# ShinobuAmasaki/forgex

Measured on NVIDIA B200. Metric: input_GBps, higher is better.
Workload: dtype u8

## Files before the change

forgex_b200/csrc/fx_cabi.cu:

```cuda
#include <cuda_runtime.h>

#include <algorithm>
#include <atomic>
#include <cstdio>
#include <cstdlib>
#include <cstring>
#include <mutex>
#include <new>
#include <string>
#include <vector>

#include "../../include/forgex_b200.h"
#include "fx_internal.hpp"
#include "fx_kernels.cuh"

using namespace fxk;

namespace {

std::atomic<long long> g_launches{0};

constexpr int STATE_CAP = 16383;
constexpr int SPARSE_STATE_CAP = 2048;
constexpr int DIRECT_LIMIT_BYTES = 40 * 1024;
// ... 470 lines not shown
        if (spt < 32) spt = 32;
        if (spt > 2048) spt = 2048;
    }
    t.spt = (int)spt;
    t.cap = (int)cap;
    t.ntiles = (n + spt - 1) / spt;
    t.smem = (size_t)tile_offset(t.table_smem, t.spt) + (size_t)extra + (size_t)t.cap + 64;
    return t;
}

template <int OP, int KIND>
int launch_ragged_t(fx_pattern* p, const Plan& pl, const uint8_t* buf, const int64_t* off, int64_t n, int64_t total,
                    uint8_t* out, cudaStream_t s, int generic) {
    auto kern = k_bool_ragged<OP, KIND>;
    Tiling t = make_tiling(pl, n, total);
    int bps = 0;
    int rc = occupancy_grid(kern, 256, t.smem, p->dev.sm_count, bps);
    if (rc) return rc;
    long long cap = (long long)p->dev.sm_count * bps;
    int grid = (int)(t.ntiles < cap ? t.ntiles : cap);
    if (grid < 1) grid = 1;
    kern<<<grid, 256, t.smem, s>>>(pl.kp, buf, off, n, total, out, t.spt, t.cap, t.ntiles, t.table_smem, generic);
    g_launches++;
    return cuda_status(cudaGetLastError());
}

template <int KIND, int NR, bool HIGH, bool TWO>
int launch_sparse_t(fx_pattern* p, const Plan& pl, const SparseParams& sp, int table_bytes, const uint8_t* buf,
                    const int64_t* off, int64_t n, int64_t total, uint8_t* out, cudaStream_t s, int64_t stride) {
    auto kern = k_in_sparse<KIND, NR, HIGH, TWO>;
    int64_t avg = n > 0 ? (total + n - 1) / n : 1;
    if (avg < 1) avg = 1;
    int64_t want = (24 * 1024) / avg;
    const int spt = (int)(want < 32 ? 32 : want > 4096 ? 4096 : want);
    const int64_t ntiles = (n + spt - 1) / spt;
    const int table_smem = KIND == 3 ? 0 : (table_bytes + 15) & ~15;
    const size_t smem = (size_t)sparse_shared_head(table_smem) + 8 * (size_t)SPARSE_WARP_BYTES;
    int bps = 0;
    int rc = occupancy_grid(kern, 256, smem, p->dev.sm_count, bps);
    if (rc) return rc;
    long long cap = (long long)p->dev.sm_count * bps;
    long long wantg = (ntiles + 7) / 8;
    int grid = (int)(wantg < cap ? wantg : cap);
    if (grid < 1) grid = 1;
    const int prezeroed = sp.start_nul == 0 && pl.kp.q0_accepting == 0;
    if (prezeroed) CUDA_TRY(cudaMemsetAsync(out, 0, (size_t)n, s));
    kern<<<grid, 256, smem, s>>>(pl.kp, sp, buf, off, n, total, out, spt, ntiles, table_smem, prezeroed, stride);
    g_launches++;
    return cuda_status(cudaGetLastError());
}

template <int KIND, bool HIGH>
int launch_sparse_k(fx_pattern* p, const Plan& pl, const SparseParams& sp, int tb, const uint8_t* buf, const int64_t* off,
                    int64_t n, int64_t total, uint8_t* out, cudaStream_t s, int64_t stride) {
    if (p->first.sweep_nr == 1 && p->first.sweep_lo[0] == p->first.sweep_hi[0]) {
        const SparseParams& one = sp;
        if (p->first.two) return launch_sparse_t<KIND, -1, HIGH, true>(p, pl, one, tb, buf, off, n, total, out, s, stride);
        return launch_sparse_t<KIND, -1, HIGH, false>(p, pl, one, tb, buf, off, n, total, out, s, stride);
    }
    switch (p->first.sweep_nr) {
        case 0: return launch_sparse_t<KIND, 0, true, false>(p, pl, sp, tb, buf, off, n, total, out, s, stride);
        case 1: return launch_sparse_t<KIND, 1, HIGH, false>(p, pl, sp, tb, buf, off, n, total, out, s, stride);
        case 2: return launch_sparse_t<KIND, 2, HIGH, false>(p, pl, sp, tb, buf, off, n, total, out, s, stride);
        case 3: return launch_sparse_t<KIND, 3, HIGH, false>(p, pl, sp, tb, buf, off, n, total, out, s, stride);
        default: return launch_sparse_t<KIND, 4, HIGH, false>(p, pl, sp, tb, buf, off, n, total, out, s, stride);
    }
}

void fill_sweep(const FirstSet& f, SparseParams& sp) {
    for (int r = 0; r < 4; r++) {
        const int k = r < f.sweep_nr ? r : 0;
        sp.add_lo[r] = (0x80u - f.sweep_lo[k]) * 0x01010101u;
        sp.add_hi[r] = (0x7Fu - f.sweep_hi[k]) * 0x01010101u;
    }
    if (f.sweep_nr == 1 && f.sweep_lo[0] == f.sweep_hi[0]) sp.add_lo[0] = f.sweep_lo[0] * 0x01010101u;
    sp.second = f.second * 0x01010101u;
    sp.second_high = f.second_high ? 0xFFFFFFFFu : 0u;
}

int launch_sparse(fx_pattern* p, const Plan& pl, const uint8_t* buf, const int64_t* off, int64_t n, int64_t total,
// ... 1107 lines not shown
```

forgex_b200/csrc/fx_kernels.cuh:

```cuda
#pragma once
#include <cuda_runtime.h>
#include <stdint.h>

namespace fxk {

static constexpr uint32_t W_ACC = 0x8000u, W_INTER = 0x4000u, W_STATE = 0x3FFFu;
static constexpr uint32_t SF_ACC = 1, SF_END = 2, SF_INTER = 4, SF_MATCHED = 8, SF_FAILACC1 = 16;

struct KParams {
    const uint16_t* table;
    const uint8_t* classmap;
    const uint8_t* flags;
    const uint8_t* lits;
    int table_words;
    int nstates;
    int row_shift;
    int start, start_nul, q0, q0_accepting;
    int all_len, pre_len, suf_len;
    int all_active;
    int pre_active, suf_active;
    const uint16_t* a_table;
    const uint8_t* a_classmap;
    const uint8_t* a_flags;
    int a_row_shift, a_start_nul, a_q0;
// ... 756 lines not shown
            if (generic || r1 == OFF_BEYOND) {
                const int64_t o0 = __ldg(offsets + c.first + i), o1 = __ldg(offsets + c.first + i + 1);
                r = eval_bool_slow<OP>(p, buf + o0, o1 - o0);
            } else {
                const int len = r1 - r0;
                const uint32_t a = tile_addr + (uint32_t)r0;
                if (degenerate_text<OP>(len, len ? lds_u8(a) : 0)) r = p.q0_accepting != 0;
                else {
                    uint32_t high = 0;
                    r = result_flag(p, walk_smem(T, (uint32_t)p.start, a, len, high));
                    if (OP == 1 && r && p.prefix_mode == 1 && (high & 0x80808080u))
                        r = recheck_in_with_prefix(p, buf + (c.base + r0), len);
                }
            }
            s_res[i] = r ? 1 : 0;
        }
        __syncthreads();
        for (int i = threadIdx.x; i < c.count; i += blockDim.x) out[c.first + i] = s_res[i];
        __syncthreads();
    }
}

struct SparseParams {
    const uint16_t* table;
    const uint8_t* classmap;
    const uint8_t* flags;
    int table_words, row_shift, q0, start_nul;
    uint32_t add_lo[4];
    uint32_t add_hi[4];
    uint32_t second;
    uint32_t second_high;
};

static constexpr int SPARSE_WARP_BYTES = 2 * 64 * 16;
static constexpr int SPARSE_PARAM_BYTES = 1024;
__host__ __device__ __forceinline__ int sparse_shared_head(int table_smem_bytes) { return ((256 + table_smem_bytes + 15) & ~15) + SPARSE_PARAM_BYTES; }

template <int NR, bool HIGH>
__device__ __forceinline__ uint32_t first_mask(const SparseParams& sp, uint32_t w) {
    uint32_t m = 0;
    if (NR == -1) {
        const uint32_t x = w ^ sp.add_lo[0];
        m = (x - 0x01010101u) & ~x;
    } else {
        const uint32_t y = w & 0x7F7F7F7Fu;
#pragma unroll
        for (int r = 0; r < NR; r++) m |= (y + sp.add_lo[r]) & ~(y + sp.add_hi[r]);
    }
    if (HIGH) m |= w;
    return m;
}
template <int NR, bool HIGH, bool TWO>
__device__ __forceinline__ uint32_t unit_any(const SparseParams& sp, const uint4& a, const uint4& b, uint32_t& seen) {
    const uint32_t w[8] = {a.x, a.y, a.z, a.w, b.x, b.y, b.z, b.w};
    const uint32_t all = w[0] | w[1] | w[2] | w[3] | w[4] | w[5] | w[6] | w[7];
    seen |= all;
    uint32_t any = 0;
    if (TWO) {
        uint32_t z2_next = 0xFFFFFFFFu;
#pragma unroll
        for (int k = 7; k >= 0; k--) {
            const uint32_t x1 = w[k] ^ sp.add_lo[0], x2 = w[k] ^ sp.second;
            uint32_t z2 = (x2 - 0x01010101u) & ~x2;
            if (!HIGH) z2 |= w[k] & sp.second_high;
            any |= (x1 - 0x01010101u) & ~x1 & __funnelshift_r(z2, z2_next, 8);
            z2_next = z2;
        }
        if (HIGH) any |= all;
    } else {
#pragma unroll
        for (int k = 0; k < 8; k++) any |= first_mask<NR, false>(sp, w[k]);
        if (HIGH) any |= all;
    }
    return any & 0x80808080u;
}
__device__ __forceinline__ uint32_t pack_byte_flags(uint32_t m) { return ((((m >> 7) & 0x01010101u) * 0x00204081u) >> 21) & 0xFu; }

template <class TBL, class FETCH>
__device__ __forceinline__ bool attempt_wins(const Anchored& A, const TBL& T, FETCH fetch, int64_t len, uint32_t st, int64_t pos) {
    uint32_t w = st;
    int64_t seq = 0;
    bool inter = false;
    for (int64_t j = pos; j <= len; j++) {
        const uint32_t b = j < len ? fetch(j) : 0u;
        if (inter && (b & 0xC0) != 0x80) {
            const uint32_t f = __ldg(A.flags + (w & W_STATE));
            if (f & ((SF_FAILACC1 << (int)(j - seq)) - SF_FAILACC1)) return true;
            inter = false;
        }
        const uint32_t nw = T.next(w & W_STATE, b);
        if ((nw & W_INTER) && !inter) seq = j;
        inter = (nw & W_INTER) != 0;
        w = nw;
        if (w & W_ACC) return true;
        if ((w & W_STATE) == 0) return false;
    }
    return false;
}

struct SparseCtx {
    const uint8_t* buf;
    const int64_t* offsets;
    int64_t stride;
    uint8_t* out;
    int64_t n, total;
    int spt;
    uint4* units;
    uint4* starts;
};
static constexpr uint32_t SPARSE_START = 0, SPARSE_RECHECK = 2;
__device__ __forceinline__ int64_t sparse_off(const int64_t* __restrict__ offsets, int64_t stride, int64_t i) {
    return offsets ? __ldg(offsets + i) : i * stride;
}

template <int KIND>
__device__ __forceinline__ Table<KIND> sparse_table(const SparseParams& sp, uint32_t s_table, uint32_t s_cmap) {
    Table<KIND> T;
    T.s_table = s_table; T.s_cmap = s_cmap; T.g_table = sp.table; T.g_cmap = sp.classmap; T.shift = sp.row_shift;
    return T;
}

template <int KIND>
__device__ __noinline__ void sparse_run_starts(const KParams& p, const SparseParams& sp, uint32_t s_table, uint32_t s_cmap,
                                               const SparseCtx& c, int count) {
    const Table<KIND> T = sparse_table<KIND>(sp, s_table, s_cmap);
    const int lane = threadIdx.x & 31;
    const Anchored A{sp.flags, sp.start_nul, sp.q0};
    __syncwarp();
    if (lane < count) {
        const uint4 e = c.starts[lane];
        const int64_t first = (int64_t)e.x * c.spt;
        const int64_t* off = c.offsets + first;
        const uint32_t kind = e.y & 7u;
        const int64_t val = (int64_t)(((unsigned long long)e.w << 32) | e.z);
        if (c.offsets == nullptr) {
            const int64_t s = kind == SPARSE_START ? val / c.stride : val;
            const uint8_t* str = c.buf + (first + s) * c.stride;
            bool win;
            if (kind == SPARSE_START) {
                win = !(c.stride == 1 && __ldg(str) == 0x20) &&
                      attempt_wins(A, T, FetchGlobal{str}, c.stride, (uint32_t)sp.q0, val - s * c.stride);
                if (win && p.prefix_mode == 1 && (e.y >> 31)) win = recheck_in_with_prefix(p, str, c.stride);
                if (win) c.out[first + s] = 1;
            } else {
                c.out[first + s] = recheck_in_with_prefix(p, str, c.stride) ? 1 : 0;
            }
        } else if (kind == SPARSE_START) {
            const int cnt = (int)((c.n - first) < c.spt ? (c.n - first) : c.spt);
            int64_t vlo = __ldg(off), vhi = __ldg(off + cnt);
            const int64_t gpos = vlo + val;
            int s = 0, sh = cnt;
            for (int iter = 0; sh - s > 1; iter++) {
                int mid = (s + sh) >> 1;
                if (iter < 6) {
                    mid = s + (int)((float)(gpos - vlo) * (float)(sh - s) / (float)(vhi - vlo));
                    mid = mid <= s ? s + 1 : mid >= sh ? sh - 1 : mid;
                }
                const int64_t v = __ldg(off + mid);
                if (v <= gpos) { s = mid; vlo = v; } else { sh = mid; vhi = v; }
            }
            const int64_t o0 = __ldg(off + s), o1 = __ldg(off + s + 1);
            const uint8_t* str = c.buf + o0;
            if (!(o1 - o0 == 1 && __ldg(str) == 0x20)) {
                bool win = attempt_wins(A, T, FetchGlobal{str}, o1 - o0, (uint32_t)sp.q0, gpos - o0);
                if (win && p.prefix_mode == 1 && (e.y >> 31)) win = recheck_in_with_prefix(p, str, o1 - o0);
                if (win) c.out[first + s] = 1;
            }
        } else {
            const int64_t o0 = __ldg(off + val), o1 = __ldg(off + val + 1);
            c.out[first + val] = recheck_in_with_prefix(p, c.buf + o0, o1 - o0) ? 1 : 0;
        }
    }
    __syncwarp();
}

template <int KIND, int NR, bool HIGH>
__device__ __noinline__ int sparse_run_units(const KParams& p, const SparseParams& sp, uint32_t s_table, uint32_t s_cmap,
                                             const SparseCtx& c, int count, int sqn) {
    const Table<KIND> T = sparse_table<KIND>(sp, s_table, s_cmap);
    const int lane = threadIdx.x & 31;
    const uint32_t FULL = 0xffffffffu;
    __syncwarp();
    uint32_t cand = 0, tile = 0, flag = 0;
    int64_t P = 0, t0 = 0;
    if (lane < count) {
        const uint4 e = c.units[lane];
        tile = e.x; flag = e.y & 0x80000000u;
        const int64_t first = (int64_t)e.x * c.spt;
        const int cnt = (int)((c.n - first) < c.spt ? (c.n - first) : c.spt);
        t0 = sparse_off(c.offsets, c.stride, first);
        const int64_t tend = sparse_off(c.offsets, c.stride, first + cnt);
        const uintptr_t gbuf = reinterpret_cast<uintptr_t>(c.buf);
        const uintptr_t ua = ((gbuf + (uintptr_t)t0) & ~(uintptr_t)31) + ((((uintptr_t)e.w << 32) | e.z) << 5);
        const uint4 v0 = __ldg(reinterpret_cast<const uint4*>(ua)), v1 = __ldg(reinterpret_cast<const uint4*>(ua + 16));
        cand = pack_byte_flags(first_mask<NR, HIGH>(sp, v0.x)) | (pack_byte_flags(first_mask<NR, HIGH>(sp, v0.y)) << 4) |
               (pack_byte_flags(first_mask<NR, HIGH>(sp, v0.z)) << 8) | (pack_byte_flags(first_mask<NR, HIGH>(sp, v0.w)) << 12) |
               (pack_byte_flags(first_mask<NR, HIGH>(sp, v1.x)) << 16) | (pack_byte_flags(first_mask<NR, HIGH>(sp, v1.y)) << 20) |
               (pack_byte_flags(first_mask<NR, HIGH>(sp, v1.z)) << 24) | (pack_byte_flags(first_mask<NR, HIGH>(sp, v1.w)) << 28);
        P = (int64_t)ua - (int64_t)gbuf;
        if (P < t0) cand &= 0xFFFFFFFFu << (int)(t0 - P);
        if (P + 32 > tend) cand &= (P >= tend) ? 0u : (0xFFFFFFFFu >> (int)(P + 32 - tend));
    }
    while (__any_sync(FULL, cand != 0)) {
        bool sv = false;
        int64_t pos = 0;
        if (cand) {
            pos = P + __ffs(cand) - 1;
            cand &= cand - 1;
            const uint32_t b = __ldg(c.buf + pos);
            const uint32_t w1 = T.next((uint32_t)sp.q0, b);
            if (w1 & (W_ACC | W_INTER)) sv = true;
            else if (w1 & W_STATE) {
                const uint32_t b1 = pos + 1 < c.total ? __ldg(c.buf + pos + 1) : 0u;
                sv = ((T.next(w1, b1) | T.next(w1, 0u)) & (W_STATE | W_ACC)) != 0;
            }
        }
        const uint32_t m = __ballot_sync(FULL, sv);
        if (m) {
            const unsigned long long rel = (unsigned long long)(pos - t0);
            if (sv) c.starts[sqn + __popc(m & ((1u << lane) - 1))] = make_uint4(tile, SPARSE_START | flag, (uint32_t)rel, (uint32_t)(rel >> 32));
            sqn += __popc(m);
            if (sqn >= 32) {
                sparse_run_starts<KIND>(p, sp, s_table, s_cmap, c, 32);
                if (lane < sqn - 32) { const uint4 x = c.starts[32 + lane]; c.starts[lane] = x; }
                sqn -= 32;
                __syncwarp();
            }
        }
    }
    __syncwarp();
    return sqn;
}

static constexpr int SPARSE_CTAS_PER_SM = 4, SPARSE_ROWS = 4;
template <int KIND, int NR, bool HIGH, bool TWO>
__global__ void __launch_bounds__(256, SPARSE_CTAS_PER_SM) k_in_sparse(KParams p, SparseParams sp, const uint8_t* __restrict__ buf,
                                                                     const int64_t* __restrict__ offsets, int64_t n, int64_t total,
                                                                     uint8_t* __restrict__ out, int spt, int64_t ntiles,
                                                                     int table_smem_bytes, int prezeroed, int64_t stride) {
    extern __shared__ __align__(128) uint8_t smem[];
    uint8_t* s_cmap = smem;
    uint8_t* s_table = smem + 256;
    const int warp = threadIdx.x >> 5, lane = threadIdx.x & 31;
    uint4* s_units = reinterpret_cast<uint4*>(smem + sparse_shared_head(table_smem_bytes) + warp * SPARSE_WARP_BYTES);
    uint4* s_starts = s_units + 64;
    KParams anch = p;
    anch.table = sp.table; anch.classmap = sp.classmap; anch.table_words = sp.table_words; anch.row_shift = sp.row_shift;
    Table<KIND> T = stage_table<KIND>(anch, s_table, s_cmap);
    static_assert(sizeof(KParams) + sizeof(SparseParams) + 8 * sizeof(SparseCtx) <= SPARSE_PARAM_BYTES, "parameter block");
    uint8_t* s_params = smem + sparse_shared_head(table_smem_bytes) - SPARSE_PARAM_BYTES;
    KParams* sh_p = reinterpret_cast<KParams*>(s_params);
    SparseParams* sh_sp = reinterpret_cast<SparseParams*>(s_params + sizeof(KParams));
    SparseCtx* sh_c = reinterpret_cast<SparseCtx*>(s_params + sizeof(KParams) + sizeof(SparseParams)) + warp;
    if (threadIdx.x == 0) { *sh_p = p; *sh_sp = sp; }
    if (lane == 0) {
        sh_c->buf = buf; sh_c->offsets = offsets; sh_c->stride = stride; sh_c->out = out; sh_c->n = n; sh_c->total = total;
        sh_c->spt = spt;
        sh_c->units = s_units; sh_c->starts = s_starts;
    }
    __syncthreads();
    const Anchored A{sp.flags, sp.start_nul, sp.q0};
    const uint32_t FULL = 0xffffffffu;
    const int nt = (int)ntiles;

    enum { ST_NEW = 0, ST_SWEEP = 1, ST_STRINGS = 2, ST_PUSH = 3 };
    int t = blockIdx.x * 8 + warp;
    int st = ST_NEW, it = 0;
    int uqn = 0, sqn = 0;
    int count = 0, nrows = 0;
    int64_t seg = 0, nunits = 0;
    uintptr_t ubase = 0;
    uint32_t hitbits = 0;
    bool high = false;
    int64_t nx0 = 0, nx1 = 0;
    bool have_next = false;

    bool drain = false;
    for (;;) {
        for (;;) {
            if (uqn >= 32 || sqn >= 32 || drain) break;
            if (st == ST_NEW) {
                if (t >= nt) { drain = true; break; }
                const int64_t first = (int64_t)t * spt;
                count = (int)((n - first) < spt ? (n - first) : spt);
                const int64_t t0 = have_next ? nx0 : sparse_off(offsets, stride, first);
                const int64_t tend = have_next ? nx1 : sparse_off(offsets, stride, first + count);
                {
                    const int64_t fn = first + (int64_t)gridDim.x * 8 * spt;
                    have_next = fn < n;
                    if (have_next) { nx0 = sparse_off(offsets, stride, fn); nx1 = sparse_off(offsets, stride, fn + spt < n ? fn + spt : n); }
                }
                const uintptr_t g0 = reinterpret_cast<uintptr_t>(buf) + (uintptr_t)t0;
                ubase = g0 & ~(uintptr_t)31;
                nunits = tend > t0 ? (int64_t)((reinterpret_cast<uintptr_t>(buf) + (uintptr_t)tend - ubase + 31) >> 5) : 0;
                seg = 0;
                high = nunits > 1024;
                st = ST_SWEEP;
            }
            if (st == ST_SWEEP) {
                const int64_t left = nunits - seg;
                nrows = (int)((left < 1024 ? left : 1024) + 31) >> 5;
                hitbits = 0;
                uint32_t seen = 0;
                for (int r = 0; r < nrows; r += SPARSE_ROWS) {
                    uint4 va[SPARSE_ROWS], vb[SPARSE_ROWS];
#pragma unroll
                    for (int k = 0; k < SPARSE_ROWS; k++) {
                        const int64_t u = seg + ((int64_t)(r + k) << 5) + lane;
                        va[k] = make_uint4(0, 0, 0, 0); vb[k] = va[k];
                        if (u < nunits && r + k < nrows) {
                            va[k] = ldg_nc_v4(reinterpret_cast<const void*>(ubase + ((uintptr_t)u << 5)));
                            vb[k] = ldg_nc_v4(reinterpret_cast<const void*>(ubase + ((uintptr_t)u << 5) + 16));
                        }
                    }
#pragma unroll
                    for (int k = 0; k < SPARSE_ROWS; k++) {
                        const int64_t u = seg + ((int64_t)(r + k) << 5) + lane;
                        const uint32_t h = (u < nunits && r + k < nrows) ? unit_any<NR, HIGH, TWO>(sp, va[k], vb[k], seen) : 0u;
                        hitbits |= (h ? 1u : 0u) << (r + k);
                    }
                }
                high = high || __any_sync(FULL, (seen & 0x80808080u) != 0);
                st = seg == 0 ? ST_STRINGS : ST_PUSH;
                it = 0;
            }
            if (st == ST_STRINGS) {
                const int64_t first = (int64_t)t * spt;
                if (prezeroed) it = count;
                while (it < count && sqn < 32) {
                    const int i = it + lane;
                    bool r = false, defer = false;
                    if (i < count) {
                        const int64_t o0 = sparse_off(offsets, stride, first + i), o1 = sparse_off(offsets, stride, first + i + 1);
                        const int64_t len = o1 - o0;
                        if (len == 0 || (len == 1 && __ldg(buf + o0) == 0x20)) r = p.q0_accepting != 0;
                        else if (sp.start_nul != 0) {
                            r = attempt_wins(A, T, FetchGlobal{buf + o0}, len, (uint32_t)sp.start_nul, 0);
                            if (r && p.prefix_mode == 1 && high) { r = false; defer = true; }
                        }
                        out[first + i] = r ? 1 : 0;
                    }
                    const uint32_t m = __ballot_sync(FULL, defer);
                    if (defer) s_starts[sqn + __popc(m & ((1u << lane) - 1))] = make_uint4((uint32_t)t, SPARSE_RECHECK, (uint32_t)i, 0u);
                    sqn += __popc(m);
                    it += 32;
                }
                if (it < count) continue;
                __syncwarp();
                st = ST_PUSH;
                it = 0;
            }
            while (it < nrows && uqn < 32) {
                const bool hit = (hitbits >> it) & 1u;
                const uint32_t m = __ballot_sync(FULL, hit);
                if (hit) {
                    const unsigned long long u = (unsigned long long)(seg + ((int64_t)it << 5) + lane);
                    s_units[uqn + __popc(m & ((1u << lane) - 1))] = make_uint4((uint32_t)t, high ? 0x80000000u : 0u, (uint32_t)u, (uint32_t)(u >> 32));
                }
                uqn += __popc(m);
                it++;
            }
            if (it < nrows) continue;
            seg += (int64_t)nrows << 5;
            if (seg < nunits) st = ST_SWEEP;
            else {
                st = ST_NEW;
                t += gridDim.x * 8;
            }
        }
        if (uqn >= 32 || (drain && uqn > 0)) {
            const int run = uqn < 32 ? uqn : 32;
            sqn = sparse_run_units<KIND, NR, HIGH>(*sh_p, *sh_sp, T.s_table, T.s_cmap, *sh_c, run, sqn);
            if (lane < uqn - run) { const uint4 x = s_units[run + lane]; s_units[lane] = x; }
            uqn -= run;
            __syncwarp();
        } else if (sqn >= 32 || (drain && sqn > 0)) {
            const int run = sqn < 32 ? sqn : 32;
            sparse_run_starts<KIND>(*sh_p, *sh_sp, T.s_table, T.s_cmap, *sh_c, run);
            if (lane < sqn - run) { const uint4 x = s_starts[run + lane]; s_starts[lane] = x; }
            sqn -= run;
            __syncwarp();
        } else {
            drain = false;
            if (st == ST_NEW && t >= nt) break;
        }
    }
}

template <int KIND>
__global__ void __launch_bounds__(256) k_regex_ragged(KParams p, const uint8_t* __restrict__ buf,
                                                      const int64_t* __restrict__ offsets, int64_t n, int64_t total,
                                                      int64_t* __restrict__ from, int64_t* __restrict__ to,
                                                      int spt, int cap, int64_t ntiles, int table_smem_bytes) {
    extern __shared__ __align__(128) uint8_t smem[];
    uint8_t* s_cmap = smem + 16;
    uint8_t* s_table = smem + 16 + 256;
    int32_t* s_off = reinterpret_cast<int32_t*>(smem + 16 + 256 + table_smem_bytes);
    uint8_t* tile = smem + tile_offset(table_smem_bytes, spt);
    const uint32_t mbar = smem_u32(smem);
    Table<KIND> T = stage_table<KIND>(p, s_table, s_cmap);
    if (threadIdx.x == 0) mbar_init(mbar, 1);
    __syncthreads();
    uint32_t phase = 0;
    const uint32_t tile_addr = smem_u32(tile);
    const bool plain = !p.all_active && !p.pre_active;
    for (int64_t t = blockIdx.x; t < ntiles; t += gridDim.x) {
        const TileCtx c = load_tile(buf, offsets, n, total, t, spt, cap, tile, s_off, mbar, phase);
        for (int i = threadIdx.x; i < c.count; i += blockDim.x) {
            const int32_t r0 = s_off[i], r1 = s_off[i + 1];
            int64_t f, e;
            if (r1 == OFF_BEYOND) {
                const int64_t o0 = __ldg(offsets + c.first + i), o1 = __ldg(offsets + c.first + i + 1);
                eval_regex(p, T, FetchGlobal{buf + o0}, o1 - o0, f, e);
            } else if (plain) {
                const int len = r1 - r0;
                const uint32_t a = tile_addr + (uint32_t)r0;
                f = 0; e = 0;
                if (!(len == 0 || (len == 1 && lds_u8(a) == 0x20))) {
                    int64_t ff, tt;
// ... 1498 lines not shown
```

Measured before the change: 3707.

## Split sparse kernel into sweeper and resolver warps linked by shared-memory rings

Restructures the sparse matcher so six warps per block only sweep input for candidate units and publish per-row hit masks into shared-memory ring buffers. The other two warps consume those slots, restage the unit bytes and offsets into shared memory, run the start attempts, and write whole-tile results. The goal is to overlap streaming with candidate resolution, cut global reloads and binary searches through global offsets, and drop the separate memset. The price is acquire/release spin-waits, a 6:2 warp split that can stall when resolvers fall behind, and a smaller maximum strings-per-tile.

Measured after the change: 1990 (median of 6 runs). -46.3%, worse.

```diff
diff --git a/forgex_b200/csrc/fx_cabi.cu b/forgex_b200/csrc/fx_cabi.cu
--- a/forgex_b200/csrc/fx_cabi.cu
+++ b/forgex_b200/csrc/fx_cabi.cu
@@ -526,20 +526,18 @@
     int64_t avg = n > 0 ? (total + n - 1) / n : 1;
     if (avg < 1) avg = 1;
     int64_t want = (24 * 1024) / avg;
-    const int spt = (int)(want < 32 ? 32 : want > 4096 ? 4096 : want);
+    const int spt = (int)(want < 32 ? 32 : want > SPARSE_MAX_SPT ? SPARSE_MAX_SPT : want);
     const int64_t ntiles = (n + spt - 1) / spt;
     const int table_smem = KIND == 3 ? 0 : (table_bytes + 15) & ~15;
-    const size_t smem = (size_t)sparse_shared_head(table_smem) + 8 * (size_t)SPARSE_WARP_BYTES;
+    const size_t smem = sparse_shared_bytes(table_smem);
     int bps = 0;
     int rc = occupancy_grid(kern, 256, smem, p->dev.sm_count, bps);
     if (rc) return rc;
     long long cap = (long long)p->dev.sm_count * bps;
-    long long wantg = (ntiles + 7) / 8;
+    long long wantg = (ntiles + SPARSE_SWEEPERS - 1) / SPARSE_SWEEPERS;
     int grid = (int)(wantg < cap ? wantg : cap);
     if (grid < 1) grid = 1;
-    const int prezeroed = sp.start_nul == 0 && pl.kp.q0_accepting == 0;
-    if (prezeroed) CUDA_TRY(cudaMemsetAsync(out, 0, (size_t)n, s));
-    kern<<<grid, 256, smem, s>>>(pl.kp, sp, buf, off, n, total, out, spt, ntiles, table_smem, prezeroed, stride);
+    kern<<<grid, 256, smem, s>>>(pl.kp, sp, buf, off, n, total, out, spt, ntiles, table_smem, stride);
     g_launches++;
     return cuda_status(cudaGetLastError());
 }
diff --git a/forgex_b200/csrc/fx_kernels.cuh b/forgex_b200/csrc/fx_kernels.cuh
--- a/forgex_b200/csrc/fx_kernels.cuh
+++ b/forgex_b200/csrc/fx_kernels.cuh
@@ -812,7 +812,6 @@
     uint32_t second_high;
 };
 
-static constexpr int SPARSE_WARP_BYTES = 2 * 64 * 16;
 static constexpr int SPARSE_PARAM_BYTES = 1024;
 __host__ __device__ __forceinline__ int sparse_shared_head(int table_smem_bytes) { return ((256 + table_smem_bytes + 15) & ~15) + SPARSE_PARAM_BYTES; }
 
@@ -878,19 +877,41 @@
     return false;
 }
 
-struct SparseCtx {
-    const uint8_t* buf;
-    const int64_t* offsets;
-    int64_t stride;
-    uint8_t* out;
-    int64_t n, total;
-    int spt;
-    uint4* units;
-    uint4* starts;
-};
-static constexpr uint32_t SPARSE_START = 0, SPARSE_RECHECK = 2;
 __device__ __forceinline__ int64_t sparse_off(const int64_t* __restrict__ offsets, int64_t stride, int64_t i) {
     return offsets ? __ldg(offsets + i) : i * stride;
+}
+
+static constexpr int SPARSE_CTAS_PER_SM = 4, SPARSE_ROWS = 4;
+static constexpr int SPARSE_SWEEPERS = 6, SPARSE_RESOLVERS = 8 - SPARSE_SWEEPERS, SPARSE_RING = 4;
+static constexpr int SPARSE_MAX_SPT = 512;
+static constexpr uint32_t SLOT_LAST = 1, SLOT_HIGH = 2;
+struct SparseSlot {
+    uint32_t tile, nrows, flags, pad;
+    int64_t seg, t0, tend;
+    uint32_t rows[32];
+};
+struct SparseRing {
+    uint32_t head, tail, done, pad;
+    SparseSlot slot[SPARSE_RING];
+};
+struct SparseResolver {
+    uint4 bytes[32 * 4];
+    int64_t off[SPARSE_MAX_SPT + 1];
+    uint16_t units[1024];
+    uint8_t res[SPARSE_MAX_SPT];
+};
+__host__ __device__ __forceinline__ size_t sparse_shared_bytes(int table_smem_bytes) {
+    return (size_t)sparse_shared_head(table_smem_bytes) + SPARSE_SWEEPERS * sizeof(SparseRing) +
+           SPARSE_RESOLVERS * sizeof(SparseResolver);
+}
+
+__device__ __forceinline__ uint32_t ld_acquire_shared(const uint32_t* p) {
+    uint32_t v;
+    asm volatile("ld.acquire.cta.shared::cta.u32 %0, [%1];" : "=r"(v) : "r"(smem_u32(p)) : "memory");
+    return v;
+}
+__device__ __forceinline__ void st_release_shared(uint32_t* p, uint32_t v) {
+    asm volatile("st.release.cta.shared::cta.u32 [%0], %1;" ::"r"(smem_u32(p)), "r"(v) : "memory");
 }
 
 template <int KIND>
@@ -900,271 +921,247 @@
     return T;
 }
 
-template <int KIND>
-__device__ __noinline__ void sparse_run_starts(const KParams& p, const SparseParams& sp, uint32_t s_table, uint32_t s_cmap,
-                                               const SparseCtx& c, int count) {
-    const Table<KIND> T = sparse_table<KIND>(sp, s_table, s_cmap);
+struct FetchUnit {
+    uint32_t a;
+    int64_t rel;
+    const uint8_t* s;
+    __device__ __forceinline__ uint32_t operator()(int64_t j) const {
+        const int64_t x = rel + j;
+        return x < 64 ? lds_u8(a + (uint32_t)x) : __ldg(s + j);
+    }
+};
+
+template <int KIND, int NR, bool HIGH>
+__device__ __forceinline__ void sparse_resolve_tile(const KParams& p, const SparseParams& sp, const Table<KIND>& T,
+                                                    const uint8_t* __restrict__ buf, const int64_t* __restrict__ offsets,
+                                                    int64_t n, int64_t total, uint8_t* __restrict__ out, int spt,
+                                                    int64_t stride, SparseRing& R, SparseResolver& W) {
     const int lane = threadIdx.x & 31;
     const Anchored A{sp.flags, sp.start_nul, sp.q0};
     __syncwarp();
-    if (lane < count) {
-        const uint4 e = c.starts[lane];
-        const int64_t first = (int64_t)e.x * c.spt;
-        const int64_t* off = c.offsets + first;
-        const uint32_t kind = e.y & 7u;
-        const int64_t val = (int64_t)(((unsigned long long)e.w << 32) | e.z);
-        if (c.offsets == nullptr) {
-            const int64_t s = kind == SPARSE_START ? val / c.stride : val;
-            const uint8_t* str = c.buf + (first + s) * c.stride;
-            bool win;
-            if (kind == SPARSE_START) {
-                win = !(c.stride == 1 && __ldg(str) == 0x20) &&
-                      attempt_wins(A, T, FetchGlobal{str}, c.stride, (uint32_t)sp.q0, val - s * c.stride);
-                if (win && p.prefix_mode == 1 && (e.y >> 31)) win = recheck_in_with_prefix(p, str, c.stride);
-                if (win) c.out[first + s] = 1;
-            } else {
-                c.out[first + s] = recheck_in_with_prefix(p, str, c.stride) ? 1 : 0;
-            }
-        } else if (kind == SPARSE_START) {
-            const int cnt = (int)((c.n - first) < c.spt ? (c.n - first) : c.spt);
-            int64_t vlo = __ldg(off), vhi = __ldg(off + cnt);
-            const int64_t gpos = vlo + val;
-            int s = 0, sh = cnt;
-            for (int iter = 0; sh - s > 1; iter++) {
-                int mid = (s + sh) >> 1;
-                if (iter < 6) {
-                    mid = s + (int)((float)(gpos - vlo) * (float)(sh - s) / (float)(vhi - vlo));
-                    mid = mid <= s ? s + 1 : mid >= sh ? sh - 1 : mid;
+    uint32_t tail = *reinterpret_cast<volatile uint32_t*>(&R.tail);
+    const SparseSlot* S = &R.slot[tail % SPARSE_RING];
+    const int64_t first = (int64_t)S->tile * spt;
+    const int count = (int)((n - first) < spt ? (n - first) : spt);
+    const int64_t t0 = S->t0, tend = S->tend;
+    const uintptr_t gbuf = reinterpret_cast<uintptr_t>(buf);
+    const uintptr_t ubase = (gbuf + (uintptr_t)t0) & ~(uintptr_t)31;
+    const uint32_t bytes_a = smem_u32(&W.bytes[lane * 4]);
+    bool staged = false;
+    for (;;) {
+        const uint32_t flags = S->flags;
+        const int64_t seg = S->seg;
+        const int nrows = (int)S->nrows;
+        int nu = 0;
+        for (int r = 0; r < nrows; r++) {
+            const uint32_t m = S->rows[r];
+            if ((m >> lane) & 1u) W.units[nu + __popc(m & ((1u << lane) - 1))] = (uint16_t)((r << 5) | lane);
+            nu += __popc(m);
+        }
+        __syncwarp();
+        tail++;
+        if (lane == 0) st_release_shared(&R.tail, tail);
+        const bool high = (flags & SLOT_HIGH) != 0;
+        for (int b = 0; b < nu || !staged; b += 32) {
+            const bool act = b + lane < nu;
+            uint4 v[4];
+            int64_t P = 0;
+#pragma unroll
+            for (int k = 0; k < 4; k++) v[k] = make_uint4(0, 0, 0, 0);
+            if (act) {
+                const uintptr_t ua = ubase + ((uintptr_t)(seg + W.units[b + lane]) << 5);
+                P = (int64_t)(ua - gbuf);
+                v[0] = __ldg(reinterpret_cast<const uint4*>(ua)); v[1] = __ldg(reinterpret_cast<const uint4*>(ua + 16));
+                if (P + 32 < total) { v[2] = __ldg(reinterpret_cast<const uint4*>(ua + 32)); v[3] = __ldg(reinterpret_cast<const uint4*>(ua + 48)); }
+            }
+            if (!staged && offsets) {
+                for (int i = lane; i <= count; i += 32) W.off[i] = __ldg(offsets + first + i);
+            }
+            uint32_t cand = 0;
+            if (act) {
+                W.bytes[lane * 4] = v[0]; W.bytes[lane * 4 + 1] = v[1]; W.bytes[lane * 4 + 2] = v[2]; W.bytes[lane * 4 + 3] = v[3];
+                cand = pack_byte_flags(first_mask<NR, HIGH>(sp, v[0].x)) | (pack_byte_flags(first_mask<NR, HIGH>(sp, v[0].y)) << 4) |
+                       (pack_byte_flags(first_mask<NR, HIGH>(sp, v[0].z)) << 8) | (pack_byte_flags(first_mask<NR, HIGH>(sp, v[0].w)) << 12) |
+                       (pack_byte_flags(first_mask<NR, HIGH>(sp, v[1].x)) << 16) | (pack_byte_flags(first_mask<NR, HIGH>(sp, v[1].y)) << 20) |
+                       (pack_byte_flags(first_mask<NR, HIGH>(sp, v[1].z)) << 24) | (pack_byte_flags(first_mask<NR, HIGH>(sp, v[1].w)) << 28);
+                if (P < t0) cand &= 0xFFFFFFFFu << (int)(t0 - P);
+                if (P + 32 > tend) cand &= (P >= tend) ? 0u : (0xFFFFFFFFu >> (int)(P + 32 - tend));
+            }
+            if (!staged) {
+                staged = true;
+                __syncwarp();
+                for (int i = lane; i < count; i += 32) {
+                    const int64_t o0 = offsets ? W.off[i] : (first + i) * stride;
+                    const int64_t len = offsets ? W.off[i + 1] - o0 : stride;
+                    bool r = false;
+                    if (len == 0) r = p.q0_accepting != 0;
+                    else if (p.q0_accepting != 0 || sp.start_nul != 0) {
+                        if (len == 1 && __ldg(buf + o0) == 0x20) r = p.q0_accepting != 0;
+                        else if (sp.start_nul != 0) {
+                            r = attempt_wins(A, T, FetchGlobal{buf + o0}, len, (uint32_t)sp.start_nul, 0);
+                            if (r && p.prefix_mode == 1 && high) r = recheck_in_with_prefix(p, buf + o0, len);
+                        }
+                    }
+                    W.res[i] = r ? 1 : 0;
                 }
-                const int64_t v = __ldg(off + mid);
-                if (v <= gpos) { s = mid; vlo = v; } else { sh = mid; vhi = v; }
-            }
-            const int64_t o0 = __ldg(off + s), o1 = __ldg(off + s + 1);
-            const uint8_t* str = c.buf + o0;
-            if (!(o1 - o0 == 1 && __ldg(str) == 0x20)) {
-                bool win = attempt_wins(A, T, FetchGlobal{str}, o1 - o0, (uint32_t)sp.q0, gpos - o0);
-                if (win && p.prefix_mode == 1 && (e.y >> 31)) win = recheck_in_with_prefix(p, str, o1 - o0);
-                if (win) c.out[first + s] = 1;
-            }
-        } else {
-            const int64_t o0 = __ldg(off + val), o1 = __ldg(off + val + 1);
-            c.out[first + val] = recheck_in_with_prefix(p, c.buf + o0, o1 - o0) ? 1 : 0;
-        }
+                __syncwarp();
+            }
+            while (cand) {
+                const int j = __ffs(cand) - 1;
+                cand &= cand - 1;
+                const int64_t pos = P + j;
+                const uint32_t b0 = lds_u8(bytes_a + j);
+                const uint32_t w1 = T.next((uint32_t)sp.q0, b0);
+                bool sv = (w1 & (W_ACC | W_INTER)) != 0;
+                if (!sv && (w1 & W_STATE)) {
+                    const uint32_t b1 = pos + 1 < total ? lds_u8(bytes_a + j + 1) : 0u;
+                    sv = ((T.next(w1, b1) | T.next(w1, 0u)) & (W_STATE | W_ACC)) != 0;
+                }
+                if (!sv) continue;
+                int s;
+                int64_t o0, len;
+                if (offsets) {
+                    int lo = 0, hi = count;
+                    while (hi - lo > 1) {
+                        const int mid = (lo + hi) >> 1;
+                        if (W.off[mid] <= pos) lo = mid; else hi = mid;
+                    }
+                    s = lo; o0 = W.off[s]; len = W.off[s + 1] - o0;
+                } else {
+                    s = (int)((pos - t0) / stride); o0 = t0 + (int64_t)s * stride; len = stride;
+                }
+                if (len == 1 && b0 == 0x20) continue;
+                bool win = attempt_wins(A, T, FetchUnit{bytes_a, o0 - P, buf + o0}, len, (uint32_t)sp.q0, pos - o0);
+                if (win && p.prefix_mode == 1 && high) win = recheck_in_with_prefix(p, buf + o0, len);
+                if (win) W.res[s] = 1;
+            }
+        }
+        if (flags & SLOT_LAST) break;
+        if (lane == 0) while (ld_acquire_shared(&R.head) == tail) __nanosleep(32);
+        __syncwarp();
+        S = &R.slot[tail % SPARSE_RING];
     }
     __syncwarp();
+    for (int i = lane; i < count; i += 32) out[first + i] = W.res[i];
+    __syncwarp();
 }
 
 template <int KIND, int NR, bool HIGH>
-__device__ __noinline__ int sparse_run_units(const KParams& p, const SparseParams& sp, uint32_t s_table, uint32_t s_cmap,
-                                             const SparseCtx& c, int count, int sqn) {
+__device__ __noinline__ void sparse_resolver(const KParams& p, const SparseParams& sp, uint32_t s_table, uint32_t s_cmap,
+                                             const uint8_t* __restrict__ buf, const int64_t* __restrict__ offsets,
+                                             int64_t n, int64_t total, uint8_t* __restrict__ out, int spt, int64_t stride,
+                                             SparseRing* rings, SparseResolver* W) {
     const Table<KIND> T = sparse_table<KIND>(sp, s_table, s_cmap);
-    const int lane = threadIdx.x & 31;
+    const int lane = threadIdx.x & 31, r = (threadIdx.x >> 5) - SPARSE_SWEEPERS;
     const uint32_t FULL = 0xffffffffu;
-    __syncwarp();
-    uint32_t cand = 0, tile = 0, flag = 0;
-    int64_t P = 0, t0 = 0;
-    if (lane < count) {
-        const uint4 e = c.units[lane];
-        tile = e.x; flag = e.y & 0x80000000u;
-        const int64_t first = (int64_t)e.x * c.spt;
-        const int cnt = (int)((c.n - first) < c.spt ? (c.n - first) : c.spt);
-        t0 = sparse_off(c.offsets, c.stride, first);
-        const int64_t tend = sparse_off(c.offsets, c.stride, first + cnt);
-        const uintptr_t gbuf = reinterpret_cast<uintptr_t>(c.buf);
-        const uintptr_t ua = ((gbuf + (uintptr_t)t0) & ~(uintptr_t)31) + ((((uintptr_t)e.w << 32) | e.z) << 5);
-        const uint4 v0 = __ldg(reinterpret_cast<const uint4*>(ua)), v1 = __ldg(reinterpret_cast<const uint4*>(ua + 16));
-        cand = pack_byte_flags(first_mask<NR, HIGH>(sp, v0.x)) | (pack_byte_flags(first_mask<NR, HIGH>(sp, v0.y)) << 4) |
-               (pack_byte_flags(first_mask<NR, HIGH>(sp, v0.z)) << 8) | (pack_byte_flags(first_mask<NR, HIGH>(sp, v0.w)) << 12) |
-               (pack_byte_flags(first_mask<NR, HIGH>(sp, v1.x)) << 16) | (pack_byte_flags(first_mask<NR, HIGH>(sp, v1.y)) << 20) |
-               (pack_byte_flags(first_mask<NR, HIGH>(sp, v1.z)) << 24) | (pack_byte_flags(first_mask<NR, HIGH>(sp, v1.w)) << 28);
-        P = (int64_t)ua - (int64_t)gbuf;
-        if (P < t0) cand &= 0xFFFFFFFFu << (int)(t0 - P);
-        if (P + 32 > tend) cand &= (P >= tend) ? 0u : (0xFFFFFFFFu >> (int)(P + 32 - tend));
-    }
-    while (__any_sync(FULL, cand != 0)) {
-        bool sv = false;
-        int64_t pos = 0;
-        if (cand) {
-            pos = P + __ffs(cand) - 1;
-            cand &= cand - 1;
-            const uint32_t b = __ldg(c.buf + pos);
-            const uint32_t w1 = T.next((uint32_t)sp.q0, b);
-            if (w1 & (W_ACC | W_INTER)) sv = true;
-            else if (w1 & W_STATE) {
-                const uint32_t b1 = pos + 1 < c.total ? __ldg(c.buf + pos + 1) : 0u;
-                sv = ((T.next(w1, b1) | T.next(w1, 0u)) & (W_STATE | W_ACC)) != 0;
-            }
-        }
-        const uint32_t m = __ballot_sync(FULL, sv);
-        if (m) {
-            const unsigned long long rel = (unsigned long long)(pos - t0);
-            if (sv) c.starts[sqn + __popc(m & ((1u << lane) - 1))] = make_uint4(tile, SPARSE_START | flag, (uint32_t)rel, (uint32_t)(rel >> 32));
-            sqn += __popc(m);
-            if (sqn >= 32) {
-                sparse_run_starts<KIND>(p, sp, s_table, s_cmap, c, 32);
-                if (lane < sqn - 32) { const uint4 x = c.starts[32 + lane]; c.starts[lane] = x; }
-                sqn -= 32;
-                __syncwarp();
-            }
-        }
-    }
-    __syncwarp();
-    return sqn;
-}
-
-static constexpr int SPARSE_CTAS_PER_SM = 4, SPARSE_ROWS = 4;
+    for (;;) {
+        bool busy = false, open = false;
+        for (int w = r; w < SPARSE_SWEEPERS; w += SPARSE_RESOLVERS) {
+            uint32_t done = 0, head = 0;
+            if (lane == 0) { done = ld_acquire_shared(&rings[w].done); head = ld_acquire_shared(&rings[w].head); }
+            done = __shfl_sync(FULL, done, 0);
+            head = __shfl_sync(FULL, head, 0);
+            if (head != *reinterpret_cast<volatile uint32_t*>(&rings[w].tail)) {
+                sparse_resolve_tile<KIND, NR, HIGH>(p, sp, T, buf, offsets, n, total, out, spt, stride, rings[w], *W);
+                busy = open = true;
+            } else if (!done) {
+                open = true;
+            }
+        }
+        if (!open) return;
+        if (!busy) __nanosleep(128);
+    }
+}
+
 template <int KIND, int NR, bool HIGH, bool TWO>
 __global__ void __launch_bounds__(256, SPARSE_CTAS_PER_SM) k_in_sparse(KParams p, SparseParams sp, const uint8_t* __restrict__ buf,
                                                                      const int64_t* __restrict__ offsets, int64_t n, int64_t total,
                                                                      uint8_t* __restrict__ out, int spt, int64_t ntiles,
-                                                                     int table_smem_bytes, int prezeroed, int64_t stride) {
+                                                                     int table_smem_bytes, int64_t stride) {
     extern __shared__ __align__(128) uint8_t smem[];
     uint8_t* s_cmap = smem;
     uint8_t* s_table = smem + 256;
     const int warp = threadIdx.x >> 5, lane = threadIdx.x & 31;
-    uint4* s_units = reinterpret_cast<uint4*>(smem + sparse_shared_head(table_smem_bytes) + warp * SPARSE_WARP_BYTES);
-    uint4* s_starts = s_units + 64;
+    SparseRing* rings = reinterpret_cast<SparseRing*>(smem + sparse_shared_head(table_smem_bytes));
+    SparseResolver* resolvers = reinterpret_cast<SparseResolver*>(rings + SPARSE_SWEEPERS);
     KParams anch = p;
     anch.table = sp.table; anch.classmap = sp.classmap; anch.table_words = sp.table_words; anch.row_shift = sp.row_shift;
-    Table<KIND> T = stage_table<KIND>(anch, s_table, s_cmap);
-    static_assert(sizeof(KParams) + sizeof(SparseParams) + 8 * sizeof(SparseCtx) <= SPARSE_PARAM_BYTES, "parameter block");
-    uint8_t* s_params = smem + sparse_shared_head(table_smem_bytes) - SPARSE_PARAM_BYTES;
-    KParams* sh_p = reinterpret_cast<KParams*>(s_params);
-    SparseParams* sh_sp = reinterpret_cast<SparseParams*>(s_params + sizeof(KParams));
-    SparseCtx* sh_c = reinterpret_cast<SparseCtx*>(s_params + sizeof(KParams) + sizeof(SparseParams)) + warp;
+    const Table<KIND> T = stage_table<KIND>(anch, s_table, s_cmap);
+    static_assert(sizeof(KParams) + sizeof(SparseParams) <= SPARSE_PARAM_BYTES, "parameter block");
+    KParams* sh_p = reinterpret_cast<KParams*>(smem + sparse_shared_head(table_smem_bytes) - SPARSE_PARAM_BYTES);
+    SparseParams* sh_sp = reinterpret_cast<SparseParams*>(sh_p + 1);
     if (threadIdx.x == 0) { *sh_p = p; *sh_sp = sp; }
-    if (lane == 0) {
-        sh_c->buf = buf; sh_c->offsets = offsets; sh_c->stride = stride; sh_c->out = out; sh_c->n = n; sh_c->total = total;
-        sh_c->spt = spt;
-        sh_c->units = s_units; sh_c->starts = s_starts;
-    }
+    if (warp < SPARSE_SWEEPERS && lane == 0) { rings[warp].head = 0; rings[warp].tail = 0; rings[warp].done = 0; }
     __syncthreads();
-    const Anchored A{sp.flags, sp.start_nul, sp.q0};
     const uint32_t FULL = 0xffffffffu;
-    const int nt = (int)ntiles;
-
-    enum { ST_NEW = 0, ST_SWEEP = 1, ST_STRINGS = 2, ST_PUSH = 3 };
-    int t = blockIdx.x * 8 + warp;
-    int st = ST_NEW, it = 0;
-    int uqn = 0, sqn = 0;
-    int count = 0, nrows = 0;
-    int64_t seg = 0, nunits = 0;
-    uintptr_t ubase = 0;
-    uint32_t hitbits = 0;
-    bool high = false;
+
+    if (warp >= SPARSE_SWEEPERS) {
+        sparse_resolver<KIND, NR, HIGH>(*sh_p, *sh_sp, T.s_table, T.s_cmap, buf, offsets, n, total, out, spt, stride, rings,
+                                        resolvers + (warp - SPARSE_SWEEPERS));
+        return;
+    }
+
+    SparseRing& R = rings[warp];
+    uint32_t head = 0;
     int64_t nx0 = 0, nx1 = 0;
     bool have_next = false;
-
-    bool drain = false;
-    for (;;) {
-        for (;;) {
-            if (uqn >= 32 || sqn >= 32 || drain) break;
-            if (st == ST_NEW) {
-                if (t >= nt) { drain = true; break; }
-                const int64_t first = (int64_t)t * spt;
-                count = (int)((n - first) < spt ? (n - first) : spt);
-                const int64_t t0 = have_next ? nx0 : sparse_off(offsets, stride, first);
-                const int64_t tend = have_next ? nx1 : sparse_off(offsets, stride, first + count);
-                {
-                    const int64_t fn = first + (int64_t)gridDim.x * 8 * spt;
-                    have_next = fn < n;
-                    if (have_next) { nx0 = sparse_off(offsets, stride, fn); nx1 = sparse_off(offsets, stride, fn + spt < n ? fn + spt : n); }
-                }
-                const uintptr_t g0 = reinterpret_cast<uintptr_t>(buf) + (uintptr_t)t0;
-                ubase = g0 & ~(uintptr_t)31;
-                nunits = tend > t0 ? (int64_t)((reinterpret_cast<uintptr_t>(buf) + (uintptr_t)tend - ubase + 31) >> 5) : 0;
-                seg = 0;
-                high = nunits > 1024;
-                st = ST_SWEEP;
-            }
-            if (st == ST_SWEEP) {
-                const int64_t left = nunits - seg;
-                nrows = (int)((left < 1024 ? left : 1024) + 31) >> 5;
-                hitbits = 0;
-                uint32_t seen = 0;
-                for (int r = 0; r < nrows; r += SPARSE_ROWS) {
-                    uint4 va[SPARSE_ROWS], vb[SPARSE_ROWS];
-#pragma unroll
-                    for (int k = 0; k < SPARSE_ROWS; k++) {
-                        const int64_t u = seg + ((int64_t)(r + k) << 5) + lane;
-                        va[k] = make_uint4(0, 0, 0, 0); vb[k] = va[k];
-                        if (u < nunits && r + k < nrows) {
-                            va[k] = ldg_nc_v4(reinterpret_cast<const void*>(ubase + ((uintptr_t)u << 5)));
-                            vb[k] = ldg_nc_v4(reinterpret_cast<const void*>(ubase + ((uintptr_t)u << 5) + 16));
-                        }
-                    }
-#pragma unroll
-                    for (int k = 0; k < SPARSE_ROWS; k++) {
-                        const int64_t u = seg + ((int64_t)(r + k) << 5) + lane;
-                        const uint32_t h = (u < nunits && r + k < nrows) ? unit_any<NR, HIGH, TWO>(sp, va[k], vb[k], seen) : 0u;
-                        hitbits |= (h ? 1u : 0u) << (r + k);
+    const int tstep = gridDim.x * SPARSE_SWEEPERS, nt = (int)ntiles;
+    for (int t = blockIdx.x * SPARSE_SWEEPERS + warp; t < nt; t += tstep) {
+        const int64_t first = (int64_t)t * spt;
+        const int count = (int)((n - first) < spt ? (n - first) : spt);
+        const int64_t t0 = have_next ? nx0 : sparse_off(offsets, stride, first);
+        const int64_t tend = have_next ? nx1 : sparse_off(offsets, stride, first + count);
+        {
+            const int64_t fn = first + (int64_t)tstep * spt;
+            have_next = fn < n;
+            if (have_next) { nx0 = sparse_off(offsets, stride, fn); nx1 = sparse_off(offsets, stride, fn + spt < n ? fn + spt : n); }
+        }
+        const uintptr_t ubase = (reinterpret_cast<uintptr_t>(buf) + (uintptr_t)t0) & ~(uintptr_t)31;
+        const int64_t nunits = tend > t0 ? (int64_t)((reinterpret_cast<uintptr_t>(buf) + (uintptr_t)tend - ubase + 31) >> 5) : 0;
+        bool high = nunits > 1024;
+        int64_t seg = 0;
+        do {
+            const int64_t left = nunits - seg;
+            const int nrows = (int)((left < 1024 ? left : 1024) + 31) >> 5;
+            uint32_t myrow = 0, seen = 0;
+            for (int r = 0; r < nrows; r += SPARSE_ROWS) {
+                uint4 va[SPARSE_ROWS], vb[SPARSE_ROWS];
+#pragma unroll
+                for (int k = 0; k < SPARSE_ROWS; k++) {
+                    const int64_t u = seg + ((int64_t)(r + k) << 5) + lane;
+                    va[k] = make_uint4(0, 0, 0, 0); vb[k] = va[k];
+                    if (u < nunits && r + k < nrows) {
+                        va[k] = ldg_nc_v4(reinterpret_cast<const void*>(ubase + ((uintptr_t)u << 5)));
+                        vb[k] = ldg_nc_v4(reinterpret_cast<const void*>(ubase + ((uintptr_t)u << 5) + 16));
                     }
                 }
-                high = high || __any_sync(FULL, (seen & 0x80808080u) != 0);
-                st = seg == 0 ? ST_STRINGS : ST_PUSH;
-                it = 0;
-            }
-            if (st == ST_STRINGS) {
-                const int64_t first = (int64_t)t * spt;
-                if (prezeroed) it = count;
-                while (it < count && sqn < 32) {
-                    const int i = it + lane;
-                    bool r = false, defer = false;
-                    if (i < count) {
-                        const int64_t o0 = sparse_off(offsets, stride, first + i), o1 = sparse_off(offsets, stride, first + i + 1);
-                        const int64_t len = o1 - o0;
-                        if (len == 0 || (len == 1 && __ldg(buf + o0) == 0x20)) r = p.q0_accepting != 0;
-                        else if (sp.start_nul != 0) {
-                            r = attempt_wins(A, T, FetchGlobal{buf + o0}, len, (uint32_t)sp.start_nul, 0);
-                            if (r && p.prefix_mode == 1 && high) { r = false; defer = true; }
-                        }
-                        out[first + i] = r ? 1 : 0;
-                    }
-                    const uint32_t m = __ballot_sync(FULL, defer);
-                    if (defer) s_starts[sqn + __popc(m & ((1u << lane) - 1))] = make_uint4((uint32_t)t, SPARSE_RECHECK, (uint32_t)i, 0u);
-                    sqn += __popc(m);
-                    it += 32;
+#pragma unroll
+                for (int k = 0; k < SPARSE_ROWS; k++) {
+                    const int64_t u = seg + ((int64_t)(r + k) << 5) + lane;
+                    const uint32_t h = (u < nunits && r + k < nrows) ? unit_any<NR, HIGH, TWO>(sp, va[k], vb[k], seen) : 0u;
+                    const uint32_t m = __ballot_sync(FULL, h != 0);
+                    if (lane == r + k) myrow = m;
                 }
-                if (it < count) continue;
-                __syncwarp();
-                st = ST_PUSH;
-                it = 0;
-            }
-            while (it < nrows && uqn < 32) {
-                const bool hit = (hitbits >> it) & 1u;
-                const uint32_t m = __ballot_sync(FULL, hit);
-                if (hit) {
-                    const unsigned long long u = (unsigned long long)(seg + ((int64_t)it << 5) + lane);
-                    s_units[uqn + __popc(m & ((1u << lane) - 1))] = make_uint4((uint32_t)t, high ? 0x80000000u : 0u, (uint32_t)u, (uint32_t)(u >> 32));
-                }
-                uqn += __popc(m);
-                it++;
-            }
-            if (it < nrows) continue;
+            }
+            high = high || __any_sync(FULL, (seen & 0x80808080u) != 0);
+            const bool last = seg + ((int64_t)nrows << 5) >= nunits;
+            if (lane == 0) while (head - ld_acquire_shared(&R.tail) >= (uint32_t)SPARSE_RING) __nanosleep(64);
+            __syncwarp();
+            SparseSlot& S = R.slot[head % SPARSE_RING];
+            if (lane < nrows) S.rows[lane] = myrow;
+            if (lane == 0) {
+                S.tile = (uint32_t)t; S.nrows = (uint32_t)nrows;
+                S.flags = (last ? SLOT_LAST : 0u) | (high ? SLOT_HIGH : 0u);
+                S.seg = seg; S.t0 = t0; S.tend = tend;
+            }
+            __syncwarp();
+            head++;
+            if (lane == 0) st_release_shared(&R.head, head);
             seg += (int64_t)nrows << 5;
-            if (seg < nunits) st = ST_SWEEP;
-            else {
-                st = ST_NEW;
-                t += gridDim.x * 8;
-            }
-        }
-        if (uqn >= 32 || (drain && uqn > 0)) {
-            const int run = uqn < 32 ? uqn : 32;
-            sqn = sparse_run_units<KIND, NR, HIGH>(*sh_p, *sh_sp, T.s_table, T.s_cmap, *sh_c, run, sqn);
-            if (lane < uqn - run) { const uint4 x = s_units[run + lane]; s_units[lane] = x; }
-            uqn -= run;
-            __syncwarp();
-        } else if (sqn >= 32 || (drain && sqn > 0)) {
-            const int run = sqn < 32 ? sqn : 32;
-            sparse_run_starts<KIND>(*sh_p, *sh_sp, T.s_table, T.s_cmap, *sh_c, run);
-            if (lane < sqn - run) { const uint4 x = s_starts[run + lane]; s_starts[lane] = x; }
-            sqn -= run;
-            __syncwarp();
-        } else {
-            drain = false;
-            if (st == ST_NEW && t >= nt) break;
-        }
-    }
+        } while (seg < nunits);
+    }
+    __syncwarp();
+    if (lane == 0) st_release_shared(&R.done, 1u);
 }
 
 template <int KIND>
```

## Tighten two-byte prefilter with pair mask, cross-unit shuffle, and unguarded sweep groups

Applied to the files above, without the earlier changes.

Rewrites the two-byte candidate test to combine the first-byte and second-byte matches before a single zero-byte detection, using a prmt-based lead-byte mask. It handles the 32-byte unit boundary by passing the neighbour's second-byte mask through a warp shuffle, and applies the same pair test when refining candidates, which should cut false-positive candidate positions. The sweep is split into full groups without bounds checks and one guarded tail group with 32-bit indexing. The cost is a shuffle per row and an extra load for the next-unit byte in the refine path.

Result: faster. 3748 before, 4137 after (median of 6 runs) (+10.4%).

```diff
diff --git a/forgex_b200/csrc/fx_kernels.cuh b/forgex_b200/csrc/fx_kernels.cuh
--- a/forgex_b200/csrc/fx_kernels.cuh
+++ b/forgex_b200/csrc/fx_kernels.cuh
@@ -830,21 +830,35 @@
     if (HIGH) m |= w;
     return m;
 }
+__device__ __forceinline__ uint32_t lead_sel(const SparseParams& sp) { return sp.second_high ? 0xBA98u : 0x4444u; }
+template <bool LEAD>
+__device__ __forceinline__ uint32_t second_zero(const SparseParams& sp, uint32_t w, uint32_t sel) {
+    uint32_t z = w ^ sp.second;
+    if (LEAD) {
+        uint32_t s;
+        asm("prmt.b32 %0, %1, 0, %2;" : "=r"(s) : "r"(w), "r"(sel));
+        z &= ~s;
+    }
+    return z;
+}
+__device__ __forceinline__ uint32_t pair_mask(const SparseParams& sp, uint32_t w, uint32_t z, uint32_t z_next) {
+    const uint32_t t = (w ^ sp.add_lo[0]) | __funnelshift_r(z, z_next, 8);
+    return (t - 0x01010101u) & ~t;
+}
 template <int NR, bool HIGH, bool TWO>
-__device__ __forceinline__ uint32_t unit_any(const SparseParams& sp, const uint4& a, const uint4& b, uint32_t& seen) {
+__device__ __forceinline__ uint32_t unit_any(const SparseParams& sp, const uint4& a, const uint4& b, uint32_t& seen,
+                                             uint32_t z_next = 0u) {
     const uint32_t w[8] = {a.x, a.y, a.z, a.w, b.x, b.y, b.z, b.w};
     const uint32_t all = w[0] | w[1] | w[2] | w[3] | w[4] | w[5] | w[6] | w[7];
     seen |= all;
     uint32_t any = 0;
     if (TWO) {
-        uint32_t z2_next = 0xFFFFFFFFu;
+        const uint32_t sel = lead_sel(sp);
 #pragma unroll
         for (int k = 7; k >= 0; k--) {
-            const uint32_t x1 = w[k] ^ sp.add_lo[0], x2 = w[k] ^ sp.second;
-            uint32_t z2 = (x2 - 0x01010101u) & ~x2;
-            if (!HIGH) z2 |= w[k] & sp.second_high;
-            any |= (x1 - 0x01010101u) & ~x1 & __funnelshift_r(z2, z2_next, 8);
-            z2_next = z2;
+            const uint32_t z = second_zero<!HIGH>(sp, w[k], sel);
+            any |= pair_mask(sp, w[k], z, z_next);
+            z_next = z;
         }
         if (HIGH) any |= all;
     } else {
@@ -954,7 +968,7 @@
     __syncwarp();
 }
 
-template <int KIND, int NR, bool HIGH>
+template <int KIND, int NR, bool HIGH, bool TWO>
 __device__ __noinline__ int sparse_run_units(const KParams& p, const SparseParams& sp, uint32_t s_table, uint32_t s_cmap,
                                              const SparseCtx& c, int count, int sqn) {
     const Table<KIND> T = sparse_table<KIND>(sp, s_table, s_cmap);
@@ -973,11 +987,23 @@
         const uintptr_t gbuf = reinterpret_cast<uintptr_t>(c.buf);
         const uintptr_t ua = ((gbuf + (uintptr_t)t0) & ~(uintptr_t)31) + ((((uintptr_t)e.w << 32) | e.z) << 5);
         const uint4 v0 = __ldg(reinterpret_cast<const uint4*>(ua)), v1 = __ldg(reinterpret_cast<const uint4*>(ua + 16));
-        cand = pack_byte_flags(first_mask<NR, HIGH>(sp, v0.x)) | (pack_byte_flags(first_mask<NR, HIGH>(sp, v0.y)) << 4) |
-               (pack_byte_flags(first_mask<NR, HIGH>(sp, v0.z)) << 8) | (pack_byte_flags(first_mask<NR, HIGH>(sp, v0.w)) << 12) |
-               (pack_byte_flags(first_mask<NR, HIGH>(sp, v1.x)) << 16) | (pack_byte_flags(first_mask<NR, HIGH>(sp, v1.y)) << 20) |
-               (pack_byte_flags(first_mask<NR, HIGH>(sp, v1.z)) << 24) | (pack_byte_flags(first_mask<NR, HIGH>(sp, v1.w)) << 28);
         P = (int64_t)ua - (int64_t)gbuf;
+        if (TWO) {
+            const uint32_t sel = lead_sel(sp);
+            uint32_t z_next = P + 32 < tend ? second_zero<true>(sp, __ldg(reinterpret_cast<const uint8_t*>(ua + 32)), sel) : 0u;
+            const uint32_t w[8] = {v0.x, v0.y, v0.z, v0.w, v1.x, v1.y, v1.z, v1.w};
+#pragma unroll
+            for (int k = 7; k >= 0; k--) {
+                const uint32_t z = second_zero<true>(sp, w[k], sel);
+                cand |= pack_byte_flags(pair_mask(sp, w[k], z, z_next) | (HIGH ? w[k] : 0u)) << (4 * k);
+                z_next = z;
+            }
+        } else {
+            cand = pack_byte_flags(first_mask<NR, HIGH>(sp, v0.x)) | (pack_byte_flags(first_mask<NR, HIGH>(sp, v0.y)) << 4) |
+                   (pack_byte_flags(first_mask<NR, HIGH>(sp, v0.z)) << 8) | (pack_byte_flags(first_mask<NR, HIGH>(sp, v0.w)) << 12) |
+                   (pack_byte_flags(first_mask<NR, HIGH>(sp, v1.x)) << 16) | (pack_byte_flags(first_mask<NR, HIGH>(sp, v1.y)) << 20) |
+                   (pack_byte_flags(first_mask<NR, HIGH>(sp, v1.z)) << 24) | (pack_byte_flags(first_mask<NR, HIGH>(sp, v1.w)) << 28);
+        }
         if (P < t0) cand &= 0xFFFFFFFFu << (int)(t0 - P);
         if (P + 32 > tend) cand &= (P >= tend) ? 0u : (0xFFFFFFFFu >> (int)(P + 32 - tend));
     }
@@ -1013,6 +1039,45 @@
 }
 
 static constexpr int SPARSE_CTAS_PER_SM = 4, SPARSE_ROWS = 4;
+
+template <int NR, bool HIGH, bool TWO, bool WHOLE>
+__device__ __forceinline__ uint32_t sweep_group(const SparseParams& sp, uintptr_t sbase, int r, int lim, uint32_t& seen) {
+    const int lane = threadIdx.x & 31;
+    uint4 va[SPARSE_ROWS], vb[SPARSE_ROWS];
+#pragma unroll
+    for (int k = 0; k < SPARSE_ROWS; k++) {
+        const int u = ((r + k) << 5) + lane;
+        const uintptr_t a = sbase + ((uintptr_t)(uint32_t)u << 5);
+        if (WHOLE || u < lim) {
+            va[k] = ldg_nc_v4(reinterpret_cast<const void*>(a));
+            vb[k] = ldg_nc_v4(reinterpret_cast<const void*>(a + 16));
+        } else {
+            va[k] = make_uint4(0, 0, 0, 0); vb[k] = va[k];
+        }
+    }
+    uint32_t zn[SPARSE_ROWS];
+    if (TWO) {
+        const uint32_t sel = lead_sel(sp);
+        uint32_t z0[SPARSE_ROWS];
+#pragma unroll
+        for (int k = 0; k < SPARSE_ROWS; k++) z0[k] = second_zero<true>(sp, va[k].x, sel);
+#pragma unroll
+        for (int k = 0; k < SPARSE_ROWS; k++) {
+            const uint32_t give = lane != 0 ? z0[k] : k + 1 < SPARSE_ROWS ? z0[k + 1] : 0u;
+            zn[k] = __shfl_sync(0xffffffffu, give, (lane + 1) & 31);
+            if (!WHOLE && ((r + k) << 5) + lane + 1 >= lim) zn[k] = 0u;
+        }
+    }
+    uint32_t bits = 0;
+#pragma unroll
+    for (int k = 0; k < SPARSE_ROWS; k++) {
+        const int u = ((r + k) << 5) + lane;
+        const uint32_t h = (WHOLE || u < lim) ? unit_any<NR, HIGH, TWO>(sp, va[k], vb[k], seen, TWO ? zn[k] : 0u) : 0u;
+        bits |= (h ? 1u : 0u) << k;
+    }
+    return bits;
+}
+
 template <int KIND, int NR, bool HIGH, bool TWO>
 __global__ void __launch_bounds__(256, SPARSE_CTAS_PER_SM) k_in_sparse(KParams p, SparseParams sp, const uint8_t* __restrict__ buf,
                                                                      const int64_t* __restrict__ offsets, int64_t n, int64_t total,
@@ -1079,27 +1144,15 @@
             }
             if (st == ST_SWEEP) {
                 const int64_t left = nunits - seg;
-                nrows = (int)((left < 1024 ? left : 1024) + 31) >> 5;
+                const int lim = (int)(left < 1024 ? left : 1024);
+                const uintptr_t sbase = ubase + ((uintptr_t)seg << 5);
+                nrows = (lim + 31) >> 5;
                 hitbits = 0;
                 uint32_t seen = 0;
-                for (int r = 0; r < nrows; r += SPARSE_ROWS) {
-                    uint4 va[SPARSE_ROWS], vb[SPARSE_ROWS];
-#pragma unroll
-                    for (int k = 0; k < SPARSE_ROWS; k++) {
-                        const int64_t u = seg + ((int64_t)(r + k) << 5) + lane;
-                        va[k] = make_uint4(0, 0, 0, 0); vb[k] = va[k];
-                        if (u < nunits && r + k < nrows) {
-                            va[k] = ldg_nc_v4(reinterpret_cast<const void*>(ubase + ((uintptr_t)u << 5)));
-                            vb[k] = ldg_nc_v4(reinterpret_cast<const void*>(ubase + ((uintptr_t)u << 5) + 16));
-                        }
-                    }
-#pragma unroll
-                    for (int k = 0; k < SPARSE_ROWS; k++) {
-                        const int64_t u = seg + ((int64_t)(r + k) << 5) + lane;
-                        const uint32_t h = (u < nunits && r + k < nrows) ? unit_any<NR, HIGH, TWO>(sp, va[k], vb[k], seen) : 0u;
-                        hitbits |= (h ? 1u : 0u) << (r + k);
-                    }
-                }
+                int r = 0;
+                for (; ((r + SPARSE_ROWS) << 5) <= lim; r += SPARSE_ROWS)
+                    hitbits |= sweep_group<NR, HIGH, TWO, true>(sp, sbase, r, lim, seen) << r;
+                if (r < nrows) hitbits |= sweep_group<NR, HIGH, TWO, false>(sp, sbase, r, lim, seen) << r;
                 high = high || __any_sync(FULL, (seen & 0x80808080u) != 0);
                 st = seg == 0 ? ST_STRINGS : ST_PUSH;
                 it = 0;
@@ -1150,7 +1203,7 @@
         }
         if (uqn >= 32 || (drain && uqn > 0)) {
             const int run = uqn < 32 ? uqn : 32;
-            sqn = sparse_run_units<KIND, NR, HIGH>(*sh_p, *sh_sp, T.s_table, T.s_cmap, *sh_c, run, sqn);
+            sqn = sparse_run_units<KIND, NR, HIGH, TWO>(*sh_p, *sh_sp, T.s_table, T.s_cmap, *sh_c, run, sqn);
             if (lane < uqn - run) { const uint4 x = s_units[run + lane]; s_units[lane] = x; }
             uqn -= run;
             __syncwarp();
```
